# ZhenghaoFei/visual_odom

Hardware: AMD Instinct MI355X
Metric: stereo frames/sec on KITTI-00 1241x376 @ ~2000 features (higher is better)
Workload: dtype u8/int32 LK (f32 2x2 solve), f64 pose solve

## Files before the change

### visual_odom_amd/csrc/capi.hip

```cpp
#include "capi_internal.h"

namespace vo_capi {

int plan_levels(vo_ctx *c, int w, int h)
{
    const int levels = plan_depth(w, h, c->prm.lk_max_level) + 1;
    int cw = w, ch = h;
    size_t off = 0;
    for (int l = 0; l < levels; l++) {
        c->lw[l] = cw;
        c->lh[l] = ch;
        c->lstride[l] = level_stride(cw);
        c->loff[l] = off;
        off += (size_t)c->lstride[l] * (ch + 2 * VO_BY);
        off = (off + 255) / 256 * 256;
        cw = (cw + 1) / 2;
        ch = (ch + 1) / 2;
    }
    c->levels = levels;
    c->img_bytes = off;
    return 0;
}

constexpr int VO_MAX_DEVICES = 64;
// ... 186 lines not shown
    c->stage_slot = (c->stage_slot + 255) / 256 * 256;
    ok = ok && o.pinned(&c->h_stage, c->stage_slot * VO_STAGE_SLOTS, hipHostMallocMapped, &c->d_stage);
    ok = ok && o.pinned(&c->h_gather, frame_gather_bytes(c->cap), hipHostMallocMapped, &c->d_gather);
    ok = ok && o.pinned(&c->h_pts_stage, sizeof(float2) * (size_t)c->cap + 16, hipHostMallocMapped, &c->d_pts_stage);
    ok = ok && o.device(&c->d_pix, c->pix_capacity);
    ok = ok && o.device(&c->d_der, c->pix_capacity);
    ok = ok && o.device(&c->d_imgs, (size_t)c->max_images);
    ok = ok && o.device(&c->d_quads, B + VO_CONST_QUADS);
    ok = ok && o.device(&c->d_pts, B * cap);
    for (int k = 0; k < 2; k++) {
        ok = ok && o.device(&c->d_trk2[k], B * 4 * cap);
        ok = ok && o.device(&c->d_status2[k], B * 4 * cap);
    }
    ok = ok && o.device(&c->d_outA, B * 5 * cap);
    ok = ok && o.device(&c->d_npts, B,  true);
    ok = ok && o.device(&c->d_nA, B,  true);
    ok = ok && o.device(&c->d_idxA, B * cap);
    ok = ok && o.device(&c->d_P, (size_t)24);
    for (auto &b : c->pb) {
        ok = ok && o.device(&b.outB, B * 4 * cap);
        ok = ok && o.device(&b.nB, B,  true);
        ok = ok && o.device(&b.idxB, B * cap);
        ok = ok && o.device(&b.xyz, B * cap * 3);
        ok = ok && o.device(&b.subsets, B * c->ransac_cap * 5);
        ok = ok && o.device(&b.inliers, B * cap);
        ok = ok && o.device(&b.models, B * c->ransac_cap * 6);
        ok = ok && o.device(&b.counts, B * c->ransac_cap);
        ok = ok && o.device(&b.results, B);
        ok = ok && o.device(&b.rstate, B);
        ok = ok && o.device(&b.epnp_ws, (size_t)epnp_ws_frames(c) * VO_EPNP_WS_HYPS * VO_EPNP_WS_DOUBLES);
        ok = ok && o.device(&b.rest_ws, (size_t)epnp_ws_frames(c) * pnp_rest_ws_doubles(c->ransac_cap));
        if (VO_DEV_MAX_POSE_WAVES >= 4)
            ok = ok && o.device(&b.epnp_gws, B * VO_EPNP_GWS_BLOCKS * VO_EPNP_UT_DOUBLES * 64);
        ok = ok && o.event(&b.ready);
        ok = ok && o.signal(&b.done);
        ok = ok && o.event(&b.tri_done);
        ok = ok && o.event(&b.em_done);
    }
    vo_default_detect_params(&c->dprm);
    c->fcap = max_pts * 4 > 16384 ? max_pts * 4 : 16384;
    if ((long long)max_w * max_h / 16 > c->fcap)
        c->fcap = (int)((long long)max_w * max_h / 16);
    ok = ok && o.device(&c->d_nmsmask, B * (size_t)max_h * ((max_w + 63) / 64));
    ok = ok && o.device(&c->d_rowcnt, B * (size_t)max_h,  true);
    ok = ok && o.device(&c->d_rowoff, B * (size_t)max_h);
    ok = ok && o.device(&c->d_detect, B,  true);
    ok = ok && o.device(&c->d_ntracked, B,  true);
    ok = ok && o.device(&c->d_nnew, B,  true);
    ok = ok && o.device(&c->d_feat, B * (size_t)c->fcap);
    ok = ok && o.device(&c->d_fages, B * (size_t)c->fcap,  true);
    ok = ok && o.pinned(&c->h_feat_stage, features_stage_bytes(c->fcap), hipHostMallocMapped, &c->d_feat_stage);
    ok = ok && o.device(&c->d_ages, B * cap,  true);
    ok = ok && o.device(&c->d_overflow, B,  true);
    for (int k = 0; k < 2; k++) {
        ok = ok && o.device(&c->d_pts_det[k], B * cap);
        ok = ok && o.device(&c->d_npts_det[k], B,  true);
        ok = ok && o.device(&c->d_ages_det[k], B * cap);
    }
    c->h_ntracked.assign(B, 0);
    c->h_detect.assign(B, 1);
    if (!ok) {
        vo_destroy(c);
        return nullptr;
    }
    c->h_npts.assign(B, 0);
    c->h_quads.assign(B, Quad{0, 0, 0, 0});
    c->img_stale.assign((size_t)c->max_images, 0);
    c->quads_cur = c->d_quads;
    if (hipMemcpy(c->d_quads + B, VO_CONST_QUAD_TABLE, sizeof(Quad) * VO_CONST_QUADS, hipMemcpyHostToDevice) != hipSuccess) {
        vo_destroy(c);
        return nullptr;
    }
    return c;
}

int vo_set_params(vo_ctx *c, const vo_params *p)
{
    if (!c || !p)
        return VO_ERR_ARG;
    if (p->lk_max_level < 0 || p->lk_max_level >= VO_MAX_LEVELS || p->ransac_iterations < 1 ||
        p->ransac_iterations > c->ransac_cap || !(p->ransac_confidence > 0 && p->ransac_confidence < 1) ||
        (p->mono_rotation && (!(p->em_prob > 0 && p->em_prob < 1) || !(p->em_threshold > 0))))
        return fail(c, VO_ERR_ARG, "vo_set_params: parameter out of range");
    if (p->input_format < VO_FMT_GRAY8 || p->input_format > VO_FMT_RGBA8)
        return fail(c, VO_ERR_ARG, "vo_set_params: input_format is not one of VO_FMT_*");
    const vo_params &q = c->prm;
    const bool rect_same = p->rectify == q.rectify &&
                           (!p->rectify || (p->rect_w == q.rect_w && p->rect_h == q.rect_h && p->rect_map_stride == q.rect_map_stride &&
                                            p->rect_map_x_left == q.rect_map_x_left && p->rect_map_y_left == q.rect_map_y_left &&
                                            p->rect_map_x_right == q.rect_map_x_right && p->rect_map_y_right == q.rect_map_y_right));
    std::vector<uint32_t> packed;
    if (!rect_same) {
        int rcr = rect_check_pack(c, p, &packed);
        if (rcr != VO_OK)
            return rcr;
    }
    const size_t raw = ((size_t)c->max_w * ingest_bpp(p->input_format) * c->max_h + 255) / 256 * 256;
    if (p->input_format != VO_FMT_GRAY8 && raw > c->stage_slot) {
        VO_HIP_TRY(c, hipSetDevice(c->device));
        int rcs = sync_all(c);
        if (rcs != VO_OK)
            return rcs;
        uint8_t *h_new = nullptr, *d_new = nullptr;
        if (!c->own.pinned(&h_new, raw * VO_STAGE_SLOTS, hipHostMallocMapped, &d_new)) {
            const hipError_t e = c->own.err;
            (void)c->own.give_back(&h_new);
// ... 839 lines not shown
```

### visual_odom_amd/csrc/capi_internal.h

```cpp
#pragma once
#include "../../include/vo_hip.h"
#include "vo_kernels.h"
#include "vo_dev_hooks.h"
#include "vo_integrate.h"
#include "vo_linalg.h"
#include "vo_rectify.h"

#include <math.h>
#include <stdio.h>
#include <stdlib.h>
#include <string.h>

#include <chrono>
#include <map>
#include <mutex>
#include <string>
#include <vector>

using namespace vo;
namespace vo {
struct CornArgs;
}
struct vocorn_params;

// ... 170 lines not shown
        vo_schedule abi() const { return vo_schedule{waves, streams, prep, wide}; }
        static Schedule from(const vo_schedule &s)
        {
            Schedule r;
            r.waves = s.pose_waves, r.streams = s.pose_streams, r.prep = s.prepare, r.wide = s.epnp_wide_frames;
            return r;
        }
    } sched;
    vo_schedule pin = {0, 0, -1, 0};
    long long sched_key[8] = {-1, 0, 0, 0, 0, 0, 0, 0};
    bool sched_probed = false;
    bool tuning = false;
    bool sync_call = false;
    struct Compare {
        Schedule list[8];
        long long key[8] = {};
        int phase = 0, left = 0, n = 0, cnt = 0;
        bool extra = false;
        hipEvent_t ev[16] = {};
        bool running() const { return phase >= 1 && phase <= cnt; }
    } cmp;
    int probe_n = 0;
    vo_schedule probe_cand[VO_PROBE_LOG_MAX] = {};
    float probe_ms[VO_PROBE_LOG_MAX] = {};
    int probe_real[VO_PROBE_LOG_MAX] = {};
    hipStream_t last_pose_stream = nullptr;
    bool quads_set = false;
    int tf_base = -1;
    struct Deferred {
        int n = 0;
        const uint8_t *img[2] = {nullptr, nullptr};
        int first = 0, stride = 0;
    } defer;
    hipEvent_t ev_t1_ready = nullptr;
    int64_t tf_gen = 0;
    bool last_run_serial = true;
    bool serial_pose = false;
    uint8_t *h_stage = nullptr, *d_stage = nullptr;
    uint8_t *h_gather = nullptr, *d_gather = nullptr;
    uint8_t *d_pts_stage = nullptr;
    uint8_t *h_feat_stage = nullptr, *d_feat_stage = nullptr;
    uint8_t *h_pts_stage = nullptr;
    size_t stage_slot = 0;
    uint32_t *d_rect_maps = nullptr;
    uint8_t *d_rect_raw = nullptr;
    RectImage *d_rect_tab = nullptr;
    size_t rect_plane = 0;
    int stage_next = 0;
    int ransac_cap = 0;
    float h_P[24] = {};
    bool have_P = false;
    std::vector<int> h_npts;
    int *d_overflow = nullptr;
    Quad *quads_cur = nullptr;
    std::vector<Quad> h_quads;
    std::vector<uint8_t> img_stale;
    struct Flow {
        bool ready = false;
        Quad *d_pairs = nullptr;
        float2 *d_next = nullptr;
        uint8_t *d_status = nullptr;
        float *d_err = nullptr;
        float2 *d_out0 = nullptr, *d_out1 = nullptr;
        int32_t *d_idx = nullptr;
        int *d_nout = nullptr;
        std::vector<Quad> h_pairs;
        int n_pairs = 0;
        int cfg[4] = {0, 0, 0, 0};
        std::vector<uint8_t> next_set;
    } flow;
    struct Corn {
        int slots = 0;
        int kcap = 0;
        unsigned *d_ints = nullptr;
        unsigned long long *d_keys = nullptr, *d_ckeys = nullptr;
        int *d_status = nullptr;
        float2 *d_pts = nullptr;
        float *d_maps = nullptr;
        int run_first = 0, run_n = 0;
        int cfg[3] = {0, 0, 0};
    } corn;
    struct CornMask {
        bool ready = false;
        uint8_t *d_masks = nullptr;
        float2 *d_kept = nullptr;
        const uint8_t **d_table = nullptr;
        std::vector<uint8_t> has;
        bool any = false;
    } cmask;
    struct Seq {
        bool on = false;
        Owner own;
        int S = 0, ring = 0, max_steps = 0;
        long long step = 0;
        Quad *d_quads = nullptr;
        int *d_active = nullptr;
        int *h_active = nullptr;
        double *d_pose = nullptr;
        double *d_traj = nullptr;
        SeqFrameInfo *d_info = nullptr;
        int *d_rows = nullptr, *d_rows_carry = nullptr, *d_nages = nullptr;
        std::vector<uint8_t> pushed, had_prev;
        std::vector<uint8_t> ever, gap;
        std::vector<int> h_rows;
        bool broken = false;
        hipEvent_t ev_upload = nullptr;
// ... 155 lines not shown
```

### visual_odom_amd/csrc/capi_run.hip

```cpp
#include "capi_internal.h"

namespace vo_capi {

int flush_deferred(vo_ctx *c, hipStream_t on)
{
    const int n = c->defer.n;
    c->defer.n = 0;
    for (int k = 0; k < n; k++) {
        int rc = upload_image(c, c->defer.first + k, c->defer.img[k], c->defer.stride, hipMemcpyHostToDevice,  true, nullptr, -1, on);
        if (rc != VO_OK)
            return rc;
    }
    return VO_OK;
}

int refuse_detect_shape(vo_ctx *c, const char *who, const char *what)
{
    if (!bucket_grid_ok(c->w, c->h, bucket_size(c), c->dprm.features_per_bucket))
        return fail(c, VO_ERR_ARG, (std::string(who) + ": bucket grid beyond the limits of the device bucketing (vo_hip.h, vo_detect_params)").c_str());
    if (c->w > 4096)
        return fail(c, VO_ERR_ARG, (std::string(who) + ": " + what + " handles images up to 4096 pixels wide").c_str());
    return VO_OK;
}

// ... 93 lines not shown
        t = t < 0 ? 0 : t > 255 ? 255 : t;
        if (ahead) {
            launch_bucket(c->d_feat, sq.d_corners + (size_t)rp * sq.S * c->fcap, c->d_fages, c->d_ntracked, c->d_nnew, c->fcap,
                          c->w, c->h, bs, fpb, c->d_pts_det[wset], c->d_ages_det[wset], c->d_npts_det[wset], cap, R.seq_active,
                          c->d_overflow, B, trk);
        } else {
            launch_detect_bucket(c->d_imgs, c->quads_cur, c->d_detect, B, c->w, c->h, t, c->dprm.fast_nonmax,
                                 c->d_nmsmask, c->d_rowcnt, c->d_rowoff, c->d_ntracked, c->d_nnew, c->fcap, c->d_feat, c->d_fages, bs, fpb,
                                 c->d_pts_det[wset], c->d_ages_det[wset], c->d_npts_det[wset], cap, R.seq_active,
                                 c->d_overflow, trk);
        }
        if (sq.on && !R.prep)
            VO_HIP_TRY(c, sq.detect.record(trk));
        c->pts_sel = wset;
        const int bound = cells * fpb < cap ? cells * fpb : cap;
        c->max_pts_set = bound;
        c->pts_on_device = true;
    }
    if (R.timed)
        VO_HIP_TRY(c, hipEventRecord(R.evs[stage_events(DET).end], trk));
    return VO_OK;
}

int run_lk(vo_ctx *c, const Run &R)
{
    vo_ctx::Seq &sq = c->seq;
    const int B = c->n_frames, cap = c->cap, wset = R.wset;
    hipStream_t trk = c->sel->stream;
    if (R.stages & VO_STAGE_LK) {
        if (R.prep)
            VO_HIP_TRY(c, hipStreamWaitEvent(trk, sq.ev_pyr, 0));
        const LkParams lp = lk_params(c);
        if (R.split) {
            const Quad &q = c->h_quads[0];
            if (c->img_stale[q.l0] | c->img_stale[q.r0])
                return fail(c, VO_ERR_STATE, "synchronous call: the t0 pair has no pyramids");
            launch_lk_hops(c->d_imgs, c->quads_cur, cur_pts(c), cur_npts(c), cap, c->max_pts_set, B, c->d_trk2[wset],
                           c->d_status2[wset], lp, 0, 1, trk);
            hipStream_t side = c->sel->filter;
            const int t1 = c->defer.first;
            int rcd = flush_deferred(c, side);
            if (rcd != VO_OK)
                return rcd;
            launch_pyramid_fused(c->d_imgs + t1, 2, c->levels, c->lw, c->lh, c->lstride, side);
            c->img_stale[t1] = c->img_stale[t1 + 1] = 0;
            VO_HIP_TRY(c, hipEventRecord(c->ev_t1_ready, side));
            VO_HIP_TRY(c, hipStreamWaitEvent(trk, c->ev_t1_ready, 0));
            if (c->img_stale[q.l1] | c->img_stale[q.r1])
                return fail(c, VO_ERR_STATE, "synchronous call: the t1 pair has no pyramids");
            launch_lk_hops(c->d_imgs, c->quads_cur, cur_pts(c), cur_npts(c), cap, c->max_pts_set, B, c->d_trk2[wset],
                           c->d_status2[wset], lp, 1, 4, trk);
        } else
            launch_lk_circular(c->d_imgs, c->quads_cur, cur_pts(c), cur_npts(c), cap, c->max_pts_set, B, c->d_trk2[wset],
                               c->d_status2[wset], lp, trk);
        c->trk_last = wset;
        c->trk_next = wset ^ 1;
        if (sq.on) {
            VO_HIP_TRY(c, sq.slot_free[(sq.step - 1) % sq.ring].record(trk));
            VO_HIP_TRY(c, sq.slot_free[sq.step % sq.ring].record(trk));
        }
    }
    if (R.timed)
        VO_HIP_TRY(c, hipEventRecord(R.evs[stage_events(LK).end], trk));
    return VO_OK;
}

int run_filter_tri(vo_ctx *c, const Run &R)
{
    vo_ctx::Seq &sq = c->seq;
    vo_ctx::PoseBufs &pb = *R.pb;
    const int B = c->n_frames, cap = c->cap;
    const bool serial = R.serial;
    hipStream_t fs = R.fs, ts = R.ts;
    c->last_run_serial = serial;
    if (R.stages & (VO_STAGE_FILTER | VO_STAGE_TRIANGULATE | VO_STAGE_PNP)) {
        if (!serial) {
            VO_HIP_TRY(c, hipEventRecord(pb.ready, c->sel->stream));
            VO_HIP_TRY(c, hipStreamWaitEvent(fs, pb.ready, 0));
        }
        VO_HIP_TRY(c, pb.done.wait(fs));
    }
    if (R.timed)
        VO_HIP_TRY(c, hipEventRecord(R.evs[stage_events(FIL).start], ts));
    if (R.stages & VO_STAGE_FILTER) {
        launch_compact(cur_pts(c), c->d_trk2[c->trk_last], c->d_status2[c->trk_last], cur_npts(c), cap,
                       c->prm.consistency_threshold, c->d_outA, c->d_idxA, c->d_nA, pb.outB, pb.idxB, pb.nB, B, fs);
        if (sq.on) {
            if (!R.dry)
                launch_seq_carry(R.seq_active, pb.outB, pb.nB, c->d_idxA, c->d_nA, cur_ages(c), cur_npts(c), cap, c->fcap,
                                 c->d_feat, c->d_fages, c->d_ntracked, c->d_overflow, sq.d_rows_carry, sq.d_nages, sq.d_info,
                                 sq.max_steps, B, fs);
            VO_HIP_TRY(c, sq.carry.record(fs));
        }
        if (!serial)
            VO_HIP_TRY(c, c->trk_free[c->trk_last].record(fs));
        if (!serial && c->pts_sel >= 0 && c->pts_sel != c->trk_last)
            VO_HIP_TRY(c, c->trk_free[c->pts_sel].record(fs));
    }
    if (R.timed)
        VO_HIP_TRY(c, hipEventRecord(R.evs[stage_events(FIL).end], ts));
    if (R.stages & VO_STAGE_TRIANGULATE)
        launch_triangulate(c->d_P, c->d_P + 12, pb.outB, pb.outB + cap, (size_t)4 * cap, pb.nB, cap,
                           c->max_pts_set, B, pb.xyz, fs);
    if (R.timed)
        VO_HIP_TRY(c, hipEventRecord(R.evs[stage_events(TRI).end], ts));
    return VO_OK;
}
// ... 113 lines not shown
```

### visual_odom_amd/csrc/dev/lk_dev.hip

```cpp
#include "../vo_kernels.h"
#include "../vo_dev_hooks.h"
#ifndef VO_HOST_EMUL
#define launch_lk_circular launch_lk_circular_product
#include "../lk.hip"
#undef launch_lk_circular
#endif

namespace vo {

__device__ __forceinline__ void half_sum2_exact_f32(int a, int b, float &fa, float &fb)
{
    VO_PERMLANE16_SWAP(a, b);
    int t = a + b;
    t = dpp_add<VO_DPP_QUAD_XOR1, 0xf>(t);
    int hi = t >> 16, lo = t & 0xffff;
    hi = dpp_add<VO_DPP_QUAD_XOR2, 0xf>(hi);
    lo = dpp_add<VO_DPP_QUAD_XOR2, 0xf>(lo);
    hi = dpp_add<VO_DPP_ROW_HALF_MIRROR, 0xf>(hi);
    lo = dpp_add<VO_DPP_ROW_HALF_MIRROR, 0xf>(lo);
    hi = dpp_add<VO_DPP_ROW_MIRROR, 0xf>(hi);
    lo = dpp_add<VO_DPP_ROW_MIRROR, 0xf>(lo);
    const float res = fmaf((float)hi, 65536.f, (float)lo);
    int x = __float_as_int(res), y = x;
    VO_PERMLANE16_SWAP(x, y);
// ... 239 lines not shown
                if (++j >= prm.max_count)
                    run = false;
                if (run) {
                    const uint32_t ua = (uint32_t)__float_as_int(nextX - fnx), ub = (uint32_t)__float_as_int(nextY - fny);
                    if ((ua > ub ? ua : ub) >= 0x3f800000u) {
                        fnx = floorf(nextX);
                        fny = floorf(nextY);
                        entry = true;
                    }
                }
            }

            if (ok && st && level == 0) {
                const int fx = vo_f2i(floorf(outX - halfWin)), fy = vo_f2i(floorf(outY - halfWin));
                if (fx < -LK_WIN || fx >= jw || fy < -LK_WIN || fy >= jh)
                    st = 0;
            }
        }

        if (act && hl == 0) {
            trk[((size_t)frame * 4 + hop) * cap + f] = make_float2(outX, outY);
            status[((size_t)frame * 4 + hop) * cap + f] = (uint8_t)st;
        }
        const bool dead = st == 0 || outX < 0.f || outY < 0.f || (hop == 0 && (p.x < 0.f || p.y < 0.f));
        if (act && dead && !prm.full_chain && hop < 3) {
            if (hl == 0)
                for (int k = hop + 1; k < 4; k++) {
                    trk[((size_t)frame * 4 + k) * cap + f] = make_float2(-1.f, -1.f);
                    status[((size_t)frame * 4 + k) * cap + f] = 0;
                }
            act = false;
        }
        if (VO_BALLOT(act) == 0ull)
            return;
        prevPtX = outX;
        prevPtY = outY;
    }
}

#ifndef VO_HOST_EMUL
static void launch_lk_circular_pair(const PyrImage *d_imgs, const Quad *d_quads, const float2 *d_pts, const int *d_npts,
                             int cap, int max_pts, int n_frames, float2 *d_trk, uint8_t *d_status,
                             const LkParams &prm, hipStream_t stream)
{
    if (max_pts <= 0 || n_frames <= 0)
        return;
    const LkGrid g = lk_grid(n_frames, (max_pts + 1) / 2);
    hipLaunchKernelGGL(lk_circular_pair_kernel, dim3((unsigned)g.blocks), dim3(64), 0, stream, d_imgs, d_quads, d_pts, d_npts, cap, n_frames,
                       g.fpg, g.ppp, d_trk, d_status, prm);
}

void launch_lk_circular(const PyrImage *d_imgs, const Quad *d_quads, const float2 *d_pts, const int *d_npts,
                        int cap, int max_pts, int n_frames, float2 *d_trk, uint8_t *d_status,
                        const LkParams &prm, hipStream_t stream)
{
    if (dev_knob("VO_LK_PAIR", 0) == 1)
        launch_lk_circular_pair(d_imgs, d_quads, d_pts, d_npts, cap, max_pts, n_frames, d_trk, d_status, prm, stream);
    else
        launch_lk_circular_product(d_imgs, d_quads, d_pts, d_npts, cap, max_pts, n_frames, d_trk, d_status, prm, stream);
}
#endif

}
```

### visual_odom_amd/csrc/lk.hip

```cpp
#include "vo_kernels.h"
#include "vo_lkmath.h"

#include <float.h>
#include <type_traits>

namespace vo {

constexpr int LK_WIN = 21;
constexpr int LK_JT_W = 48, LK_JT_H = 40;
constexpr int LK_W_BITS = 14;
template <int W>
struct LkWin {
    static_assert(W % 2 == 1 && W >= 5 && W <= LK_WIN, "odd windows of 5 .. 21: the pyramid's borders are laid out for 21");
    static constexpr int SEGS = (W + 6) / 7, LANES = W * SEGS, COLS = 7 * SEGS + 1, ROWS = W + 1, LAST = W - 7 * (SEGS - 1);
    static constexpr int OFF_X = ((LK_JT_W - COLS) / 2) & ~3, OFF_Y = (LK_JT_H - ROWS) / 2;
    static_assert(LANES <= 64 && LK_JT_W >= COLS + OFF_X + 3 && LK_JT_H >= ROWS + OFF_Y, "the lane map and the tile hold the window");
};
constexpr uint32_t lk_seg_mask(int valid, int m)
{
    return (2 * m < valid ? 0x0000ffffu : 0u) | (2 * m + 1 < valid ? 0xffff0000u : 0u);
}

template <bool COLS>
__device__ __forceinline__ void lk_weights_packed(float a, float b, uint32_t &w0, uint32_t &w1)
{
    const float s = (float)(1 << LK_W_BITS), magic = 12582912.f;
    typedef float F32x2 __attribute__((vector_size(8)));
    const F32x2 p = {a, b}, q = 1.f - p, pswap = {b, a};
    const F32x2 x = q * pswap;
    const uint32_t r00 = (uint32_t)__float_as_int(fmaf(q[0] * q[1], s, magic));
    const uint32_t r01 = (uint32_t)__float_as_int(fmaf(x[1], s, magic));
    const uint32_t r10 = (uint32_t)__float_as_int(fmaf(x[0], s, magic));
    const uint32_t iw11 = ((1u << LK_W_BITS) + 3u * 0x4B400000u) - (r00 + r01 + r10);
    w0 = perm_b32(COLS ? r10 : r01, r00, VO_SEL_LO16);
    w1 = perm_b32(iw11, COLS ? r01 : r10, VO_SEL_LO16);
}
__device__ __forceinline__ void lk_weights(float a, float b, uint32_t &wt, uint32_t &wb)
{
    lk_weights_packed<false>(a, b, wt, wb);
}
__device__ __forceinline__ void lk_weights_cols(float a, float b, uint32_t &wl, uint32_t &wr)
{
    lk_weights_packed<true>(a, b, wl, wr);
}

struct LkOrigin {
    int x, y;
};
template <int W = LK_WIN>
__device__ __forceinline__ bool lk_tile_misses(bool have_tile, int jx0, int jy0, int inx, int iny)
{
    return !have_tile || inx < jx0 || inx + LkWin<W>::COLS > jx0 + LK_JT_W || iny < jy0 || iny + LkWin<W>::ROWS > jy0 + LK_JT_H;
}
template <int W = LK_WIN>
// ... 30 lines not shown
#ifndef VO_HOST_EMUL
    asm volatile("" : "+v"(lane));
#endif
    const int row = (lane * 43) >> 7, col = lane - CPR * row;
    const uint32_t g0 = (uint32_t)(row * jstride + 16 * col);
    const int next_col = 21 * jstride + 16, next_row = 22 * jstride - 16 * (CPR - 1);
    const uint32_t g1 = g0 + (uint32_t)(col == CPR - 1 ? next_row : next_col);
    const bool second = lane < CHUNKS - 64;
    const U32x4A4 v0 = *(const VO_GLOBAL U32x4A4 *)(tb + g0);
    U32x4A4 v1 = v0;
    if (second)
        v1 = *(const VO_GLOBAL U32x4A4 *)(tb + g1);
    *reinterpret_cast<uint4 *>(&tile[16 * lane]) = make_uint4(v0.a, v0.b, v0.c, v0.d);
    if (second)
        *reinterpret_cast<uint4 *>(&tile[16 * lane + 1024]) = make_uint4(v1.a, v1.b, v1.c, v1.d);
    return org;
}
template <int W = LK_WIN>
__device__ __forceinline__ LkOrigin lk_tile_cover(uint8_t *tile, const VO_GLOBAL uint8_t *__restrict__ Jimg, int jstride, int jx_max, int jy_max,
                                              int inx, int iny, int lane, bool have_tile, int jx0, int jy0)
{
    if (!lk_tile_misses<W>(have_tile, jx0, jy0, inx, iny))
        return LkOrigin{jx0, jy0};
    __syncthreads();
    const LkOrigin o = lk_tile_refill_wave<W>(tile, Jimg, jstride, jx_max, jy_max, inx, iny, lane);
    __syncthreads();
    return o;
}
__device__ __forceinline__ void lk_cell_rows(const uint8_t *tile, int off, uint32_t Jt[7], uint32_t Jb[7])
{
    const U32x2A1 t = *reinterpret_cast<const U32x2A1 *>(&tile[off]);
    const U32x2A1 u = *reinterpret_cast<const U32x2A1 *>(&tile[off + LK_JT_W]);
    lift7(t.a, t.b, Jt);
    lift7(u.a, u.b, Jb);
}
__device__ __forceinline__ void lk_cell_cols(const uint8_t *tile, int off, uint32_t Jc[8])
{
    const U32x2A1 t = *reinterpret_cast<const U32x2A1 *>(&tile[off]);
    const U32x2A1 u = *reinterpret_cast<const U32x2A1 *>(&tile[off + LK_JT_W]);
    lift8_cols(t.a, t.b, u.a, u.b, Jc);
}

#ifndef VO_LK_ATTRS
#define VO_LK_ATTRS __launch_bounds__(64, 7)
#endif
constexpr int VO_LK_USE_INITIAL_FLOW = 4, VO_LK_GET_MIN_EIGENVALS = 8;
template <bool SPLIT, bool ERR, int WIN = LK_WIN, bool FLAGS = false>
__device__ __forceinline__ void lk_circular_body(const PyrImage *__restrict__ imgs, const Quad *__restrict__ quads,
                                                 const float2 *__restrict__ pts_in, const int *__restrict__ n_pts, int cap,
                                                 int n_frames, int fpg , int ppp ,
                                                 float2 *__restrict__ trk,
                                                 uint8_t *__restrict__ status,
                                                 const LkParams prm, int hop_begin, int hop_end, float *__restrict__ err = nullptr,
                                                 int flags = 0)
{
    __shared__ __attribute__((aligned(16))) uint8_t s_jt[LK_JT_H * LK_JT_W];

    const int bid = blockIdx.x;
    const int xcd = bid & 7, slot = bid >> 3;
    const int grp = slot / ppp, fi = slot - grp * ppp;
    const int frame = grp * fpg + (xcd & (fpg - 1));
    const int f = (xcd / fpg) * ppp + fi;
    if (frame >= n_frames || f >= n_pts[frame])
        return;
    const int lane = threadIdx.x;
    using LW = LkWin<WIN>;
    const bool live = lane < LW::LANES;
    const int lr = live ? lane : LW::LANES - 1;
    const int r = lr / LW::SEGS, c0 = 7 * (lr - LW::SEGS * r);
    const int lane_off = r * LK_JT_W + c0;

    const Quad q = quads[frame];
    const float halfWin = (WIN - 1) * 0.5f;
    const float FLT_SCALE = 1.f / (1 << 20);
    const float eps_lo = (float)(prm.epsilon * 0.999999), eps_hi = (float)(prm.epsilon * 1.000001);
    const float min_eig_n = prm.min_eig * (1.001f * (float)(2 * WIN * WIN));

    const float2 p = pts_in[(size_t)frame * cap + f];
    float prevPtX = unif(p.x), prevPtY = unif(p.y);
    if (SPLIT && hop_begin > 0) {
        const size_t o = ((size_t)frame * 4 + (hop_begin - 1)) * cap + f;
        const float2 q0 = trk[o];
        const bool dead0 = status[o] == 0 || q0.x < 0.f || q0.y < 0.f || (hop_begin == 1 && (p.x < 0.f || p.y < 0.f));
        if (dead0 && !prm.full_chain)
            return;
        prevPtX = unif(q0.x);
        prevPtY = unif(q0.y);
    }

    for (int hop = SPLIT ? hop_begin : 0; hop < (ERR ? 1 : SPLIT ? hop_end : 4); hop++) {
        const int pi = hop == 0 ? q.l0 : hop == 1 ? q.r0 : hop == 2 ? q.r1 : q.l1;
        const int ni = hop == 0 ? q.r0 : hop == 1 ? q.r1 : hop == 2 ? q.l1 : q.l0;
        const PyrImage &I = imgs[pi];
        const PyrImage &J = imgs[ni];
        float outX = prm.max_level >= 0 ? prevPtX : 0.f, outY = prm.max_level >= 0 ? prevPtY : 0.f;
        if constexpr (FLAGS) {
            if ((flags & VO_LK_USE_INITIAL_FLOW) && prm.max_level >= 0) {
                const float2 g = trk[(size_t)frame * cap + f];
                outX = unif(g.x);
                outY = unif(g.y);
            }
        }
        int st = 1;
        float errv = 0.f;

        for (int level = prm.max_level; level >= 0; level--) {
            const float scale = __int_as_float((127 - level) << 23);
            float prevX = prevPtX * scale, prevY = prevPtY * scale;
            const float start = __int_as_float(level == prm.max_level ? (127 - level) << 23 : 0x40000000);
            outX *= start;
            outY *= start;
// ... 244 lines not shown
                            } else
                                e = udot2(pk_absdiff_i16(Jp[m], Ipe[m]), 0x00010001u, e);
                        }
                        errv = wave_sum_exact_f32(live ? (int)e : 0) / (float)(32 * WIN * WIN);
                    }
                }
            }
        }

        if constexpr (ERR) {
            if (lane == 0) {
                trk[(size_t)frame * cap + f] = make_float2(outX, outY);
                status[(size_t)frame * cap + f] = (uint8_t)st;
                if (err != nullptr) {
                    if constexpr (FLAGS)
                        err[(size_t)frame * cap + f] = ((flags & VO_LK_GET_MIN_EIGENVALS) || st) ? errv : 0.f;
                    else
                        err[(size_t)frame * cap + f] = st ? errv : 0.f;
                }
            }
            return;
        }
        if (lane == 0) {
            trk[((size_t)frame * 4 + hop) * cap + f] = make_float2(outX, outY);
            status[((size_t)frame * 4 + hop) * cap + f] = (uint8_t)st;
        }
        const bool dead = st == 0 || outX < 0.f || outY < 0.f || (hop == 0 && (p.x < 0.f || p.y < 0.f));
        if (dead && !prm.full_chain && hop < 3) {
            if (lane == 0)
                for (int k = hop + 1; k < 4; k++) {
                    trk[((size_t)frame * 4 + k) * cap + f] = make_float2(-1.f, -1.f);
                    status[((size_t)frame * 4 + k) * cap + f] = 0;
                }
            return;
        }
        prevPtX = unif(outX);
        prevPtY = unif(outY);
    }
}

__global__ VO_LK_ATTRS void lk_circular_kernel(const PyrImage *__restrict__ imgs,
                                                          const Quad *__restrict__ quads,
                                                          const float2 *__restrict__ pts_in,
                                                          const int *__restrict__ n_pts, int cap,
                                                          int n_frames, int fpg ,
                                                          int ppp ,
                                                          float2 *__restrict__ trk,
                                                          uint8_t *__restrict__ status,
                                                          LkParams prm)
{
    lk_circular_body<false, false>(imgs, quads, pts_in, n_pts, cap, n_frames, fpg, ppp, trk, status, prm, 0, 4);
}

__global__ VO_LK_ATTRS void lk_hops_kernel(const PyrImage *__restrict__ imgs, const Quad *__restrict__ quads,
                                           const float2 *__restrict__ pts_in, const int *__restrict__ n_pts, int cap,
                                           int n_frames, int fpg, int ppp, float2 *__restrict__ trk,
                                           uint8_t *__restrict__ status, LkParams prm, int hop_begin, int hop_end)
{
    lk_circular_body<true, false>(imgs, quads, pts_in, n_pts, cap, n_frames, fpg, ppp, trk, status, prm, hop_begin, hop_end);
}

#ifndef VO_LK_FLOW_ATTRS
#define VO_LK_FLOW_ATTRS __launch_bounds__(64, 6)
#endif
__global__ VO_LK_FLOW_ATTRS void lk_flow_kernel(const PyrImage *__restrict__ imgs, const Quad *__restrict__ pairs,
                                                const float2 *__restrict__ pts_in, const int *__restrict__ n_pts, int cap,
                                                int n_frames, int fpg, int ppp, float2 *__restrict__ next,
                                                uint8_t *__restrict__ status,
                                                float *__restrict__ err , LkParams prm)
{
    lk_circular_body<false, true>(imgs, pairs, pts_in, n_pts, cap, n_frames, fpg, ppp, next, status, prm, 0, 1, err);
}

template <int W>
__global__ VO_LK_FLOW_ATTRS void lk_flow_win_kernel(const PyrImage *__restrict__ imgs, const Quad *__restrict__ pairs,
                                                    const float2 *__restrict__ pts_in, const int *__restrict__ n_pts, int cap,
                                                    int n_frames, int fpg, int ppp, float2 *__restrict__ next,
                                                    uint8_t *__restrict__ status,
                                                    float *__restrict__ err , LkParams prm)
{
    static_assert(W < LK_WIN, "21 is lk_flow_kernel");
    lk_circular_body<false, true, W>(imgs, pairs, pts_in, n_pts, cap, n_frames, fpg, ppp, next, status, prm, 0, 1, err);
}

template <int W>
__global__ VO_LK_FLOW_ATTRS void lk_flow_flags_kernel(const PyrImage *__restrict__ imgs, const Quad *__restrict__ pairs,
                                                      const float2 *__restrict__ pts_in, const int *__restrict__ n_pts, int cap,
                                                      int n_frames, int fpg, int ppp, float2 *__restrict__ next,
                                                      uint8_t *__restrict__ status,
                                                      float *__restrict__ err , LkParams prm, int flags)
{
    lk_circular_body<false, true, W, true>(imgs, pairs, pts_in, n_pts, cap, n_frames, fpg, ppp, next, status, prm, 0, 1, err, flags);
}

struct LkGrid {
    int fpg, ppp, blocks;
};
inline LkGrid lk_grid(int n_frames, int n_items)
{
    const int fpg = n_frames >= 8 ? 8 : n_frames >= 4 ? 4 : n_frames >= 2 ? 2 : 1;
    const int parts = 8 / fpg, ppp = (n_items + parts - 1) / parts;
    const int groups = (n_frames + fpg - 1) / fpg;
    return {fpg, ppp, 8 * groups * ppp};
}

template <int... W, typename F>
inline bool lk_visit_window(int win, F &&f)
{
    return ((win == W && (f(std::integral_constant<int, W>{}), true)) || ...);
}
template <typename F>
inline bool lk_for_window(int win, F &&f)
{
    return lk_visit_window<5, 7, 9, 11, 13, 15, 17, 19, LK_WIN>(win, f);
}

template <int W, typename R>
inline void lk_flow_route(int flags, R &&run)
{
    if (flags != 0)
        run(lk_flow_flags_kernel<W>, flags);
    else if constexpr (W == LK_WIN)
        run(lk_flow_kernel);
    else
        run(lk_flow_win_kernel<W>);
}

#ifndef VO_HOST_EMUL
void launch_lk_flow(int win, int flags, const PyrImage *d_imgs, const Quad *d_pairs, const float2 *d_pts, const int *d_npts, int cap,
                    int max_pts, int n_frames, float2 *d_next, uint8_t *d_status, float *d_err, const LkParams &prm, hipStream_t stream)
{
    if (max_pts <= 0 || n_frames <= 0 || (flags & ~(VO_LK_USE_INITIAL_FLOW | VO_LK_GET_MIN_EIGENVALS)))
        return;
    const LkGrid g = lk_grid(n_frames, max_pts);
    lk_for_window(win, [&](auto w) {
        lk_flow_route<decltype(w)::value>(flags, [&](auto kernel, auto... tail) {
            hipLaunchKernelGGL(kernel, dim3((unsigned)g.blocks), dim3(64), 0, stream, d_imgs, d_pairs, d_pts, d_npts, cap, n_frames, g.fpg,
                               g.ppp, d_next, d_status, d_err, prm, tail...);
        });
    });
}

void launch_lk_circular(const PyrImage *d_imgs, const Quad *d_quads, const float2 *d_pts, const int *d_npts,
                        int cap, int max_pts, int n_frames, float2 *d_trk, uint8_t *d_status,
                        const LkParams &prm, hipStream_t stream)
{
    if (max_pts <= 0 || n_frames <= 0)
        return;
    const LkGrid g = lk_grid(n_frames, max_pts);
    hipLaunchKernelGGL(lk_circular_kernel, dim3((unsigned)g.blocks), dim3(64), 0, stream, d_imgs, d_quads, d_pts, d_npts, cap,
                       n_frames, g.fpg, g.ppp, d_trk, d_status, prm);
}

void launch_lk_hops(const PyrImage *d_imgs, const Quad *d_quads, const float2 *d_pts, const int *d_npts, int cap, int max_pts,
                    int n_frames, float2 *d_trk, uint8_t *d_status, const LkParams &prm, int hop_begin, int hop_end,
                    hipStream_t stream)
{
    if (max_pts <= 0 || n_frames <= 0 || hop_begin < 0 || hop_end > 4 || hop_begin >= hop_end)
        return;
    const LkGrid g = lk_grid(n_frames, max_pts);
    hipLaunchKernelGGL(lk_hops_kernel, dim3((unsigned)g.blocks), dim3(64), 0, stream, d_imgs, d_quads, d_pts, d_npts, cap, n_frames,
                       g.fpg, g.ppp, d_trk, d_status, prm, hop_begin, hop_end);
}

#endif

}

#ifdef VO_HOST_EMUL
#include "dev/lk_dev.hip"
#endif
```

### visual_odom_amd/csrc/vo_kernels.h

```cpp
#pragma once

#include "../../include/vo_hip.h"
#include "vo_dev.h"

namespace vo {

constexpr int ingest_bpp(int fmt) { return fmt == VO_FMT_GRAY8 ? 1 : fmt == VO_FMT_GRAY8_X2 ? 2 : fmt <= VO_FMT_RGB8 ? 3 : 4; }

inline int align_up(int v, int a) { return (v + a - 1) / a * a; }
inline int level_stride(int w) { return align_up(VO_BX + w + VO_BY, 16); }
inline int plan_depth(int w, int h, int lk_max_level)
{
    int l = 0;
    for (int cw = w, ch = h;; l++) {
        const int nw = (cw + 1) / 2, nh = (ch + 1) / 2;
        if (l == lk_max_level || l + 1 >= VO_MAX_LEVELS || nw <= 21 || nh <= 21)
            break;
        cw = nw;
        ch = nh;
    }
    return l;
}

struct LkParams {
    int max_level;
    int max_count;
    double epsilon;
    float min_eig;
    int full_chain;
};

struct PnpParams {
    int iters;
    float reproj;
    double confidence;
    float K[9];
};

struct PnpResult {
    double rvec[3], tvec[3], R[9];
    int n_inliers;
    int status;
    int niters;
    int best_iter;
    int max_good;
    int lm_iters;
};

struct RansacState {
    int it;
    int niters;
    int max_good;
    int best;
    uint64_t rng;
    int arrive;
    int pad_;
// ... 14 lines not shown
    int niters;
    int best;
};

struct SeqFrameInfo {
    int n_bucketed;
    int n_circ;
    int n_tracked;
    int n_inliers;
    int pnp_status;
    int flags;
    int ransac_iters;
    int overflow;
};
struct SeqTail {
    const int *active = nullptr;
    const EmResult *em = nullptr;
    double *pose = nullptr;
    double *traj = nullptr;
    SeqFrameInfo *info = nullptr;
    int *n_rows = nullptr;
    int max_steps = 0;
};
struct SeqIngest {
    const uint8_t *left, *right;
    int stride, image0;
};
struct RectImage {
    const uint8_t *raw;
    int image, side;
};

constexpr int VO_EPNP_UT_DOUBLES = 144 + 12, VO_EPNP_GWS_BLOCKS = 2;
constexpr int VO_EPNP_WS_DOUBLES = 288, VO_EPNP_WS_HYPS = 128, VO_EPNP_WS_MAX_FRAMES = 16, VO_EPNP_SPLIT_DEFAULT_FRAMES = 4;
inline int pnp_rest_groups(int iters) { return iters > VO_EPNP_WS_HYPS ? (iters - VO_EPNP_WS_HYPS + 63) / 64 : 1; }
inline size_t pnp_rest_ws_doubles(int iters) { return (size_t)pnp_rest_groups(iters) * VO_EPNP_UT_DOUBLES * 64; }

#ifndef VO_HOST_EMUL
struct EmBufs {
    double2 *q0 = nullptr, *q1 = nullptr;
    int32_t *subsets = nullptr;
    RansacState *rstate = nullptr;
    double *models = nullptr;
    int *nmodels = nullptr;
    int *counts = nullptr;
    double *bestE = nullptr;
    uint8_t *mask = nullptr;
};

void launch_pyramid_fused(const PyrImage *d_imgs, int n_images, int n_levels, const int *lw, const int *lh, const int *lstride,
                          hipStream_t stream);
void launch_pull_image(const void *src_pinned_dev, void *dst, size_t bytes, hipStream_t stream, const void *pts_pinned_dev = nullptr,
                       void *pts_dst = nullptr, int n_pts = 0, int *count_dst = nullptr);
void launch_lk_circular(const PyrImage *d_imgs, const Quad *d_quads, const float2 *d_pts, const int *d_npts,
                        int cap, int max_pts, int n_frames, float2 *d_trk, uint8_t *d_status,
                        const LkParams &prm, hipStream_t stream);
void launch_lk_hops(const PyrImage *d_imgs, const Quad *d_quads, const float2 *d_pts, const int *d_npts, int cap, int max_pts,
                    int n_frames, float2 *d_trk, uint8_t *d_status, const LkParams &prm, int hop_begin, int hop_end,
                    hipStream_t stream);
void launch_lk_flow(int win, int flags, const PyrImage *d_imgs, const Quad *d_pairs, const float2 *d_pts, const int *d_npts, int cap,
                    int max_pts, int n_frames, float2 *d_next, uint8_t *d_status, float *d_err, const LkParams &prm, hipStream_t stream);
void launch_detect_bucket(const PyrImage *d_imgs, const Quad *d_quads, const int *d_detect, int n_frames, int w,
                          int h, int threshold, int nonmax, unsigned long long *d_nmsmask,
                          int *d_rowcnt, int *d_rowoff,
                          const int *d_ntracked, int *d_nnew, int cap, float2 *d_feat, const int *d_ages,
                          int bucket_size, int fpb, float2 *d_out_pts, int *d_out_ages, int *d_out_n, int out_cap,
                          const int *d_active, int *d_overflow, hipStream_t stream);
void launch_fast_corners(const PyrImage *d_imgs, const Quad *d_quads, const int *d_detect, int n_frames, int w, int h,
                         int threshold, int nonmax, unsigned long long *d_nmsmask, int *d_rowcnt, int *d_rowoff,
                         const int *d_ntracked, int *d_nnew, int cap, float2 *d_out, hipStream_t stream);
bool bucket_grid_ok(int w, int h, int bucket_size, int fpb);
void launch_bucket(const float2 *d_feat, const float2 *d_corners, const int *d_ages, const int *d_ntracked,
                   const int *d_nnew, int cap, int w, int h, int bucket_size, int fpb, float2 *d_out_pts, int *d_out_ages,
                   int *d_out_n, int out_cap, const int *d_active, int *d_overflow, int n_frames, hipStream_t stream);
void launch_seq_ingest(const SeqIngest *tab, int n_pairs, int w, int h, int pitch, uint8_t *pix0, size_t img_bytes,
                       bool over_pcie, hipStream_t stream);
int launch_seq_ingest_fmt(int fmt, const SeqIngest *tab, int n_pairs, int w, int h, int pitch, uint8_t *pix0, size_t img_bytes,
                          bool over_pcie, hipStream_t stream);
int launch_pull_image_fmt(int fmt, const void *src, int src_stride, void *dst, int pitch, int w, int h, hipStream_t stream,
                          const void *pts_pinned_dev = nullptr, void *pts_dst = nullptr, int n_pts = 0, int *count_dst = nullptr);
void launch_rectify(const RectImage *tab, int n_images, int w, int h, int raw_pitch, const uint32_t *maps, int pitch, uint8_t *pix0,
                    size_t img_bytes, hipStream_t stream);
void launch_seq_prepare(const int *active, const int *n_tracked, int redetect_below, int *detect,
                        const int *n_corners, int *n_new, int n_seq, hipStream_t stream);
void launch_seq_carry(const int *active, const float2 *outB, const int *nB, const int *idxA, const int *nA,
                      const int *ages, const int *n_bucketed, int cap, int fcap, float2 *feat, int *fages,
                      int *n_tracked, const int *overflow, int *n_rows_carry, int *n_ages, SeqFrameInfo *info,
                      int max_steps, int n_seq, hipStream_t stream);
constexpr size_t VO_GATHER_HEADER = 512;
struct FrameGatherLayout {
    size_t cap;
    static constexpr size_t n_circ = 0, n_out = 4, has_em = 8, pnp = 16, em = 256;
    constexpr size_t row(int k) const { return VO_GATHER_HEADER + (size_t)k * cap * sizeof(float2); }
    constexpr size_t xyz() const { return row(4); }
    constexpr size_t keep_idx() const { return xyz() + cap * 3 * sizeof(float); }
    constexpr size_t keep_idx_circ() const { return keep_idx() + cap * sizeof(int32_t); }
    constexpr size_t inliers() const { return keep_idx_circ() + cap * sizeof(int32_t); }
    constexpr size_t bytes() const { return inliers() + cap * sizeof(int32_t); }
};
static_assert(FrameGatherLayout::pnp + sizeof(PnpResult) <= FrameGatherLayout::em, "the PnpResult lies in bytes 16 .. 256 of the header");
static_assert(FrameGatherLayout::em + sizeof(EmResult) <= VO_GATHER_HEADER, "the EmResult lies in bytes 256 .. 512 of the header");
struct FrameGather {
    const int *nA, *nB;
    const float2 *outB;
    const float *xyz;
    const int32_t *idxB, *idxA, *inliers;
    const PnpResult *result;
    const EmResult *em;
    int cap;
// ... 90 lines not shown
```

Before: 25260.

## Add per-XCD atomic work queues with stealing to LK circular tracking kernel

Adds a work-queue variant of the circular LK kernel. Each block draws its work item from one of eight per-XCD atomic counters and steals from the other queues once its own runs dry, so blocks are no longer bound to a fixed blockIdx mapping. The aim is to balance load across XCDs and CUs when per-point iteration counts differ. In exchange it launches surplus blocks, adds atomics, and double-buffers the counters so the next launch's set is reset in the kernel; it only applies when there are at least 16 frames.

```diff
diff --git a/visual_odom_amd/csrc/capi.hip b/visual_odom_amd/csrc/capi.hip
--- a/visual_odom_amd/csrc/capi.hip
+++ b/visual_odom_amd/csrc/capi.hip
@@ -262,6 +262,7 @@
     ok = ok && o.pinned(&c->h_feat_stage, features_stage_bytes(c->fcap), hipHostMallocMapped, &c->d_feat_stage);
     ok = ok && o.device(&c->d_ages, B * cap,  true);
     ok = ok && o.device(&c->d_overflow, B,  true);
+    ok = ok && o.device(&c->lk_queues.d_next, (size_t)LKQ_WORDS,  true);
     for (int k = 0; k < 2; k++) {
         ok = ok && o.device(&c->d_pts_det[k], B * cap);
         ok = ok && o.device(&c->d_npts_det[k], B,  true);
diff --git a/visual_odom_amd/csrc/capi_internal.h b/visual_odom_amd/csrc/capi_internal.h
--- a/visual_odom_amd/csrc/capi_internal.h
+++ b/visual_odom_amd/csrc/capi_internal.h
@@ -246,6 +246,7 @@
     bool have_P = false;
     std::vector<int> h_npts;
     int *d_overflow = nullptr;
+    LkQueues lk_queues;
     Quad *quads_cur = nullptr;
     std::vector<Quad> h_quads;
     std::vector<uint8_t> img_stale;
diff --git a/visual_odom_amd/csrc/capi_run.hip b/visual_odom_amd/csrc/capi_run.hip
--- a/visual_odom_amd/csrc/capi_run.hip
+++ b/visual_odom_amd/csrc/capi_run.hip
@@ -169,7 +169,7 @@
                            c->d_status2[wset], lp, 1, 4, trk);
         } else
             launch_lk_circular(c->d_imgs, c->quads_cur, cur_pts(c), cur_npts(c), cap, c->max_pts_set, B, c->d_trk2[wset],
-                               c->d_status2[wset], lp, trk);
+                               c->d_status2[wset], lp, trk, &c->lk_queues);
         c->trk_last = wset;
         c->trk_next = wset ^ 1;
         if (sq.on) {
diff --git a/visual_odom_amd/csrc/dev/lk_dev.hip b/visual_odom_amd/csrc/dev/lk_dev.hip
--- a/visual_odom_amd/csrc/dev/lk_dev.hip
+++ b/visual_odom_amd/csrc/dev/lk_dev.hip
@@ -315,12 +315,12 @@
 
 void launch_lk_circular(const PyrImage *d_imgs, const Quad *d_quads, const float2 *d_pts, const int *d_npts,
                         int cap, int max_pts, int n_frames, float2 *d_trk, uint8_t *d_status,
-                        const LkParams &prm, hipStream_t stream)
+                        const LkParams &prm, hipStream_t stream, LkQueues *queues)
 {
     if (dev_knob("VO_LK_PAIR", 0) == 1)
         launch_lk_circular_pair(d_imgs, d_quads, d_pts, d_npts, cap, max_pts, n_frames, d_trk, d_status, prm, stream);
     else
-        launch_lk_circular_product(d_imgs, d_quads, d_pts, d_npts, cap, max_pts, n_frames, d_trk, d_status, prm, stream);
+        launch_lk_circular_product(d_imgs, d_quads, d_pts, d_npts, cap, max_pts, n_frames, d_trk, d_status, prm, stream, queues);
 }
 #endif
 
diff --git a/visual_odom_amd/csrc/lk.hip b/visual_odom_amd/csrc/lk.hip
--- a/visual_odom_amd/csrc/lk.hip
+++ b/visual_odom_amd/csrc/lk.hip
@@ -1,5 +1,6 @@
 #include "vo_kernels.h"
 #include "vo_lkmath.h"
+#include "vo_lkqueue.h"
 
 #include <float.h>
 #include <type_traits>
@@ -136,11 +137,10 @@
                                                  float2 *__restrict__ trk,
                                                  uint8_t *__restrict__ status,
                                                  const LkParams prm, int hop_begin, int hop_end, float *__restrict__ err = nullptr,
-                                                 int flags = 0)
+                                                 int flags = 0, int bid = blockIdx.x )
 {
     __shared__ __attribute__((aligned(16))) uint8_t s_jt[LK_JT_H * LK_JT_W];
 
-    const int bid = blockIdx.x;
     const int xcd = bid & 7, slot = bid >> 3;
     const int grp = slot / ppp, fi = slot - grp * ppp;
     const int frame = grp * fpg + (xcd & (fpg - 1));
@@ -491,6 +491,52 @@
     lk_circular_body<false, false>(imgs, quads, pts_in, n_pts, cap, n_frames, fpg, ppp, trk, status, prm, 0, 4);
 }
 
+__device__ __forceinline__ unsigned lk_queue_draw(unsigned *next, int q)
+{
+#ifdef VO_HOST_EMUL
+    unsigned t = 0;
+    if (threadIdx.x == 0)
+        t = next[LKQ_STRIDE * q]++;
+#else
+    unsigned t = 0;
+    if (threadIdx.x == 0)
+        t = __hip_atomic_fetch_add(&next[LKQ_STRIDE * q], 1u, __ATOMIC_RELAXED, __HIP_MEMORY_SCOPE_AGENT);
+#endif
+    return (unsigned)uni((int)t);
+}
+__device__ __forceinline__ void lk_queue_mark(unsigned *next, int q)
+{
+    unsigned t = 0;
+#ifdef VO_HOST_EMUL
+    if (threadIdx.x == 0)
+        next[LKQ_STRIDE * q] |= LKQ_ALL_DRY;
+    (void)uni((int)t);
+#else
+    if (threadIdx.x == 0)
+        t = __hip_atomic_fetch_or(&next[LKQ_STRIDE * q], LKQ_ALL_DRY, __ATOMIC_RELAXED, __HIP_MEMORY_SCOPE_AGENT);
+    asm volatile("" ::"s"(uni((int)t)));
+#endif
+}
+__global__ VO_LK_ATTRS void lk_circular_queue_kernel(const PyrImage *__restrict__ imgs, const Quad *__restrict__ quads,
+                                                     const float2 *__restrict__ pts_in, const int *__restrict__ n_pts, int cap,
+                                                     int n_frames, int fpg , int ppp, float2 *__restrict__ trk,
+                                                     uint8_t *__restrict__ status, LkParams prm, int items ,
+                                                     unsigned *next, unsigned *other)
+{
+    if (blockIdx.x == 0 && threadIdx.x < (unsigned)LKQ_QUEUES) {
+#ifdef VO_HOST_EMUL
+        other[LKQ_STRIDE * threadIdx.x] = 0u;
+#else
+        __hip_atomic_store(&other[LKQ_STRIDE * threadIdx.x], 0u, __ATOMIC_RELAXED, __HIP_MEMORY_SCOPE_AGENT);
+#endif
+    }
+    const int bid = lk_queue_take((int)(blockIdx.x & 7), items, [&](int q) { return lk_queue_draw(next, q); },
+                                  [&](int q) { lk_queue_mark(next, q); });
+    if (bid < 0)
+        return;
+    lk_circular_body<false, false>(imgs, quads, pts_in, n_pts, cap, n_frames, fpg, ppp, trk, status, prm, 0, 4, nullptr, 0, bid);
+}
+
 __global__ VO_LK_ATTRS void lk_hops_kernel(const PyrImage *__restrict__ imgs, const Quad *__restrict__ quads,
                                            const float2 *__restrict__ pts_in, const int *__restrict__ n_pts, int cap,
                                            int n_frames, int fpg, int ppp, float2 *__restrict__ trk,
@@ -582,10 +628,20 @@
 
 void launch_lk_circular(const PyrImage *d_imgs, const Quad *d_quads, const float2 *d_pts, const int *d_npts,
                         int cap, int max_pts, int n_frames, float2 *d_trk, uint8_t *d_status,
-                        const LkParams &prm, hipStream_t stream)
+                        const LkParams &prm, hipStream_t stream, LkQueues *queues)
 {
     if (max_pts <= 0 || n_frames <= 0)
         return;
+    if (queues != nullptr && queues->d_next != nullptr && n_frames >= LKQ_MIN_FRAMES &&
+        (long long)((n_frames + 7) / 8) * max_pts < (1ll << 26)) {
+        const LkQueueGrid g = lk_queue_grid(n_frames, max_pts);
+        const int set = queues->launches++ & 1;
+        unsigned *const cur = queues->d_next + set * (LKQ_QUEUES * LKQ_STRIDE);
+        unsigned *const oth = queues->d_next + (set ^ 1) * (LKQ_QUEUES * LKQ_STRIDE);
+        hipLaunchKernelGGL(lk_circular_queue_kernel, dim3((unsigned)g.blocks), dim3(64), 0, stream, d_imgs, d_quads, d_pts, d_npts, cap,
+                           n_frames, g.fpg, g.ppp, d_trk, d_status, prm, g.items, cur, oth);
+        return;
+    }
     const LkGrid g = lk_grid(n_frames, max_pts);
     hipLaunchKernelGGL(lk_circular_kernel, dim3((unsigned)g.blocks), dim3(64), 0, stream, d_imgs, d_quads, d_pts, d_npts, cap,
                        n_frames, g.fpg, g.ppp, d_trk, d_status, prm);
diff --git a/visual_odom_amd/csrc/vo_kernels.h b/visual_odom_amd/csrc/vo_kernels.h
--- a/visual_odom_amd/csrc/vo_kernels.h
+++ b/visual_odom_amd/csrc/vo_kernels.h
@@ -2,6 +2,7 @@
 
 #include "../../include/vo_hip.h"
 #include "vo_dev.h"
+#include "vo_lkqueue.h"
 
 namespace vo {
 
@@ -122,9 +123,13 @@
                           hipStream_t stream);
 void launch_pull_image(const void *src_pinned_dev, void *dst, size_t bytes, hipStream_t stream, const void *pts_pinned_dev = nullptr,
                        void *pts_dst = nullptr, int n_pts = 0, int *count_dst = nullptr);
+struct LkQueues {
+    unsigned *d_next = nullptr;
+    unsigned launches = 0;
+};
 void launch_lk_circular(const PyrImage *d_imgs, const Quad *d_quads, const float2 *d_pts, const int *d_npts,
                         int cap, int max_pts, int n_frames, float2 *d_trk, uint8_t *d_status,
-                        const LkParams &prm, hipStream_t stream);
+                        const LkParams &prm, hipStream_t stream, LkQueues *queues = nullptr);
 void launch_lk_hops(const PyrImage *d_imgs, const Quad *d_quads, const float2 *d_pts, const int *d_npts, int cap, int max_pts,
                     int n_frames, float2 *d_trk, uint8_t *d_status, const LkParams &prm, int hop_begin, int hop_end,
                     hipStream_t stream);
diff --git a/visual_odom_amd/csrc/vo_lkqueue.h b/visual_odom_amd/csrc/vo_lkqueue.h
--- /dev/null
+++ b/visual_odom_amd/csrc/vo_lkqueue.h
@@ -0,0 +1,56 @@
+#pragma once
+
+#include "vo_isa.h"
+
+namespace vo {
+
+constexpr int LKQ_QUEUES = 8;
+constexpr int LKQ_STRIDE = 32;
+constexpr int LKQ_SETS = 2;
+constexpr int LKQ_WORDS = LKQ_SETS * LKQ_QUEUES * LKQ_STRIDE;
+constexpr int LKQ_MIN_FRAMES = 16;
+#ifndef VO_LKQ_SURPLUS_DIV
+#define VO_LKQ_SURPLUS_DIV 16
+#endif
+constexpr int LKQ_SURPLUS_DIV = VO_LKQ_SURPLUS_DIV;
+constexpr unsigned LKQ_ALL_DRY = 1u << 30;
+
+struct LkItem {
+    int frame, f;
+};
+VO_HD LkItem lk_block_item(int bid, int fpg, int ppp)
+{
+    const int xcd = bid & 7, slot = bid >> 3;
+    const int grp = slot / ppp, fi = slot - grp * ppp;
+    return LkItem{grp * fpg + (xcd & (fpg - 1)), (xcd / fpg) * ppp + fi};
+}
+
+template <typename Draw, typename Mark>
+VO_HD int lk_queue_take(int x, int items, Draw &&draw, Mark &&mark)
+{
+    unsigned t = draw(x);
+    if (t < (unsigned)items)
+        return LKQ_QUEUES * (int)t + x;
+    if (t >= LKQ_ALL_DRY)
+        return -1;
+    for (int k = 1; k < LKQ_QUEUES; k++) {
+        const int q = (x + k) & (LKQ_QUEUES - 1);
+        t = draw(q);
+        if (t < (unsigned)items)
+            return LKQ_QUEUES * (int)t + q;
+    }
+    mark(x);
+    return -1;
+}
+
+struct LkQueueGrid {
+    int fpg, ppp, items, surplus, blocks;
+};
+inline LkQueueGrid lk_queue_grid(int n_frames, int n_items, int surplus_div = LKQ_SURPLUS_DIV)
+{
+    const int groups = (n_frames + 7) / 8, items = groups * n_items;
+    const int surplus = (items + surplus_div - 1) / surplus_div;
+    return {8, n_items, items, surplus, LKQ_QUEUES * (items + surplus)};
+}
+
+}
```

Result: faster. 25580 (median of 6 runs) (+1.3%).
